# constantinpape/torch-em

Measured on AMD Instinct MI355X. Metric: voxels/sec fwd+bwd, UNet3d 1x128^3 bs=2, higher is better.
Workload: dtype f32-class (forward convs on normalised activations: fp32 operands split into 2 fp16 terms = 22 mantissa bits, lo plane scaled by 2^12 with its own fp32 accumulator, 3 fp16 MFMAs per product; other forward convs 3 bf16 terms / 6 MFMAs; data-gradient convs 2 bf16 terms / 3 MFMAs (16-bit products); WEI

## Files before the change

torch_em_amd/csrc/capi.hip:

```cpp
#include "tem_common.h"
#include "conv_internal.h"
#include "tem_act.h"
#include <stdarg.h>
#include <string.h>

static thread_local char g_err[512] = "";

void tem_set_error(const char* fmt, ...) {
    va_list ap;
    va_start(ap, fmt);
    vsnprintf(g_err, sizeof(g_err), fmt, ap);
    va_end(ap);
}

extern "C" const char* tem_last_error(void) { return g_err; }

struct TemOption {
    const char* name;
    long long def;
};
static const TemOption g_opt_table[TEM_OPT_COUNT] = {
    {"wgrad_zs", 3},
    {"wgrad_zs_persist", 1},
    {"wgrad_sums", 1},
    {"wgrad_sums_min_mb", 128},
    {"fwd_persistent", -1},
    {"conv_fwd_variant", -1},
    {"conv1x1_stream", 1},
    {"fwd_ksplit_chunks", 0},
    {"wgrad_cus", 256},
    {"upsample_generic", 0},
    {"team_min_units", 0},
    {"zr_splitk", 1},
    {"zr_wide", 1},
    {"zr_tile_blocks", 1},
    {"dice_vox", 1},
    {"upsample2_ch8", 1},
    {"pool_vec8", 2},
    {"fp32_zr", 1},
    {"zr_pair", 1},
};
static long long g_opt_val[TEM_OPT_COUNT];
static bool g_opt_set[TEM_OPT_COUNT];

long long tem_option(int id) {
    if (id < 0 || id >= TEM_OPT_COUNT) return 0;
    return __atomic_load_n(&g_opt_set[id], __ATOMIC_RELAXED) ? __atomic_load_n(&g_opt_val[id], __ATOMIC_RELAXED)
                                                            : g_opt_table[id].def;
}
static int opt_find(const char* name) {
    if (!name) return -1;
    for (int i = 0; i < TEM_OPT_COUNT; ++i)
        if (!strcmp(name, g_opt_table[i].name)) return i;
    return -1;
}
extern "C" int tem_set_option(const char* name, int64_t value) {
    const int id = opt_find(name);
    TEM_REQUIRE(id >= 0, "tem_set_option: unknown option '%s'", name ? name : "(null)");
    __atomic_store_n(&g_opt_val[id], (long long)value, __ATOMIC_RELAXED);
    __atomic_store_n(&g_opt_set[id], true, __ATOMIC_RELAXED);
    return TEM_OK;
}
extern "C" int tem_get_option(const char* name, int64_t* value) {
    const int id = opt_find(name);
    TEM_REQUIRE(id >= 0 && value, "tem_get_option: unknown option '%s'", name ? name : "(null)");
    *value = (int64_t)tem_option(id);
    return TEM_OK;
}
extern "C" int tem_version(void) { return 100; }

extern "C" int tem_device_cus(void) {
    int dev = 0;
    if (hipGetDevice(&dev) != hipSuccess) return TEM_ELAUNCH;
    hipDeviceProp_t prop;
    if (hipGetDeviceProperties(&prop, dev) != hipSuccess) return TEM_ELAUNCH;
    return prop.multiProcessorCount;
}
int tem_ncu() {
    static int ncu = 0;
    if (!ncu) {
        ncu = tem_device_cus();
        if (ncu <= 0) ncu = 256;
    }
    return ncu;
}

#define TT_V 64
#define TT_C 32

__global__ __launch_bounds__(256) void k_nchw_to_nhwc(const float* __restrict__ src, float* __restrict__ dst,
                                                      int64_t dst_ld, int C, int64_t V, int64_t vtiles, int ctiles) {
    __shared__ float tile[TT_C][TT_V + 1];
    int64_t ntiles = vtiles * ctiles;
    int n = blockIdx.y;
    for (int64_t t = blockIdx.x; t < ntiles; t += gridDim.x) {
        int ct = (int)(t % ctiles);
        int64_t vt = t / ctiles;
        int64_t v0 = vt * TT_V;
        int c0 = ct * TT_C;
        for (int i = threadIdx.x; i < TT_C * TT_V; i += 256) {
            int c = i / TT_V, v = i % TT_V;
            float val = 0.f;
            if (c0 + c < C && v0 + v < V) val = src[((int64_t)n * C + c0 + c) * V + v0 + v];
            tile[c][v] = val;
        }
        __syncthreads();
        for (int i = threadIdx.x; i < TT_C * TT_V; i += 256) {
            int v = i / TT_C, c = i % TT_C;
            if (c0 + c < C && v0 + v < V) dst[((int64_t)n * V + v0 + v) * dst_ld + c0 + c] = tile[c][v];
        }
        __syncthreads();
    }
}

__global__ __launch_bounds__(256) void k_nhwc_to_nchw(const float* __restrict__ src, int64_t src_ld,
                                                      float* __restrict__ dst, int C, int64_t V, int64_t vtiles,
                                                      int ctiles) {
    __shared__ float tile[TT_C][TT_V + 1];
    int64_t ntiles = vtiles * ctiles;
    int n = blockIdx.y;
    for (int64_t t = blockIdx.x; t < ntiles; t += gridDim.x) {
        int ct = (int)(t % ctiles);
        int64_t vt = t / ctiles;
        int64_t v0 = vt * TT_V;
        int c0 = ct * TT_C;
        for (int i = threadIdx.x; i < TT_C * TT_V; i += 256) {
            int v = i / TT_C, c = i % TT_C;
            float val = 0.f;
            if (c0 + c < C && v0 + v < V) val = src[((int64_t)n * V + v0 + v) * src_ld + c0 + c];
            tile[c][v] = val;
        }
        __syncthreads();
        for (int i = threadIdx.x; i < TT_C * TT_V; i += 256) {
            int c = i / TT_V, v = i % TT_V;
            if (c0 + c < C && v0 + v < V) dst[((int64_t)n * C + c0 + c) * V + v0 + v] = tile[c][v];
        }
        __syncthreads();
    }
}

extern "C" int tem_nchw_to_nhwc(const float* src, float* dst, int64_t dst_ld, int N, int C, int64_t V,
                                tem_stream_t stream) {
    TEM_REQUIRE(src && dst && N > 0 && C > 0 && V > 0 && dst_ld >= C, "tem_nchw_to_nhwc: bad arguments");
    int64_t vtiles = tem_cdiv(V, TT_V);
    int ctiles = (int)tem_cdiv(C, TT_C);
    int64_t nt = vtiles * ctiles;
    dim3 grid((unsigned)(nt > 4096 ? 4096 : nt), N);
    hipLaunchKernelGGL(k_nchw_to_nhwc, grid, dim3(256), 0, (hipStream_t)stream, src, dst, dst_ld, C, V, vtiles, ctiles);
    TEM_CHECK_LAUNCH("tem_nchw_to_nhwc");
    return TEM_OK;
}

extern "C" int tem_nhwc_to_nchw(const float* src, int64_t src_ld, float* dst, int N, int C, int64_t V,
                                tem_stream_t stream) {
    TEM_REQUIRE(src && dst && N > 0 && C > 0 && V > 0 && src_ld >= C, "tem_nhwc_to_nchw: bad arguments");
    int64_t vtiles = tem_cdiv(V, TT_V);
    int ctiles = (int)tem_cdiv(C, TT_C);
    int64_t nt = vtiles * ctiles;
    dim3 grid((unsigned)(nt > 4096 ? 4096 : nt), N);
    hipLaunchKernelGGL(k_nhwc_to_nchw, grid, dim3(256), 0, (hipStream_t)stream, src, src_ld, dst, C, V, vtiles, ctiles);
    TEM_CHECK_LAUNCH("tem_nhwc_to_nchw");
    return TEM_OK;
}

#define STD_BLOCKS 256

__global__ __launch_bounds__(256) void k_std_partial(const float* __restrict__ x, int64_t L, double* __restrict__ part) {
    int n = blockIdx.y;
    const float* row = x + (int64_t)n * L;
    double s = 0.0, ss = 0.0;
    for (int64_t i = (int64_t)blockIdx.x * 256 + threadIdx.x; i < L; i += (int64_t)gridDim.x * 256) {
        double v = (double)row[i];
        s += v;
        ss += v * v;
    }
    s = tem_wave_sum_d(s);
    ss = tem_wave_sum_d(ss);
    __shared__ double sh[2][4];
    int w = threadIdx.x >> 6;
    if ((threadIdx.x & 63) == 0) { sh[0][w] = s; sh[1][w] = ss; }
    __syncthreads();
    if (threadIdx.x == 0) {
        part[((int64_t)n * gridDim.x + blockIdx.x) * 2 + 0] = sh[0][0] + sh[0][1] + sh[0][2] + sh[0][3];
        part[((int64_t)n * gridDim.x + blockIdx.x) * 2 + 1] = sh[1][0] + sh[1][1] + sh[1][2] + sh[1][3];
    }
}

__global__ __launch_bounds__(256) void k_std_apply(const float* __restrict__ x, float* __restrict__ y, int64_t L,
                                                   const double* __restrict__ part, int nblk, float eps) {
    int n = blockIdx.y;
    __shared__ float sh_mean, sh_inv;
    if (threadIdx.x == 0) {
        double s = 0.0, ss = 0.0;
// ... 49 lines not shown
```

torch_em_amd/csrc/pool_upsample.hip:

```cpp
#include "tem_common.h"
#include "tem_act.h"

template <int VEC>
struct VecT;
template <>
struct VecT<4> {
    typedef float4 type;
};
template <>
struct VecT<1> {
    typedef float type;
};

template <int VEC, typename T>
__device__ __forceinline__ void ld_vec(const T* p, float (&v)[VEC]) {
    if constexpr (VEC == 8) {
        act_ld8(p, v);
    } else if constexpr (VEC == 4) {
        const float4 t = act_ld4(p);
        v[0] = t.x; v[1] = t.y; v[2] = t.z; v[3] = t.w;
    } else {
        v[0] = act_ld1(p);
    }
}
// ... 744 lines not shown
    if constexpr (CH == 8) act_st8(p, a.v);
    else act_st4(p, make_float4(a.v[0], a.v[1], a.v[2], a.v[3]));
}
template <int CH>
__device__ __forceinline__ FV<CH> fv_zero() {
    FV<CH> r;
#pragma unroll
    for (int j = 0; j < CH; ++j) r.v[j] = 0.f;
    return r;
}
template <int CH>
__device__ __forceinline__ FV<CH> lerp2(float l0, const FV<CH>& a, float l1, const FV<CH>& b) {
    FV<CH> r;
#pragma unroll
    for (int j = 0; j < CH; ++j) r.v[j] = l0 * a.v[j] + l1 * b.v[j];
    return r;
}

template <int FZ, typename T, int CH = 4>
__global__ __launch_bounds__(256) void k_upsample2_fwd(const T* __restrict__ x, int64_t x_ld, T* __restrict__ y,
                                                       int64_t y_ld, int D, int H, int W, int C,
                                                       float* __restrict__ part) {
    extern __shared__ float lsu[];
    const int Ho = 2 * H, Wo = 2 * W;
    const int cq = C / CH;
    int row = blockIdx.x;
    const int yi = row % H;
    row /= H;
    const int zi = row % D;
    const int n = row / D;
    const int ym = max(yi - 1, 0), yp = min(yi + 1, H - 1);
    const int zm = max(zi - 1, 0), zp = min(zi + 1, D - 1);
    const float ya0 = yi == 0 ? 1.f : 0.25f, ya1 = yi == 0 ? 0.f : 0.75f;
    const float za0 = zi == 0 ? 1.f : 0.25f, za1 = zi == 0 ? 0.f : 0.75f;
    const int zrow[3] = {zm, zi, zp}, yrow[3] = {ym, yi, yp};
    float s1[CH], s2[CH];
#pragma unroll
    for (int j = 0; j < CH; ++j) s1[j] = s2[j] = 0.f;
    for (int i = threadIdx.x; i < W * cq; i += 256) {
        const int xi = i / cq, c0 = (i % cq) * CH;
        const int xm = max(xi - 1, 0), xp = min(xi + 1, W - 1);
        const float xa0 = xi == 0 ? 1.f : 0.25f, xa1 = xi == 0 ? 0.f : 0.75f;
        FV<CH> Y[FZ == 2 ? 3 : 1][2][2];
#pragma unroll
        for (int kz = 0; kz < (FZ == 2 ? 3 : 1); ++kz) {
            const int zc = FZ == 2 ? zrow[kz] : zi;
            FV<CH> X[3][2];
#pragma unroll
            for (int ky = 0; ky < 3; ++ky) {
                const T* r = x + ((((int64_t)n * D + zc) * H + yrow[ky]) * W) * x_ld + c0;
                const FV<CH> a = ldv<CH>(r + (int64_t)xm * x_ld), b = ldv<CH>(r + (int64_t)xi * x_ld), c = ldv<CH>(r + (int64_t)xp * x_ld);
                X[ky][0] = lerp2(xa0, a, xa1, b);
                X[ky][1] = lerp2(0.75f, b, 0.25f, c);
            }
#pragma unroll
            for (int sx = 0; sx < 2; ++sx) {
                Y[kz][0][sx] = lerp2(ya0, X[0][sx], ya1, X[1][sx]);
                Y[kz][1][sx] = lerp2(0.75f, X[1][sx], 0.25f, X[2][sx]);
            }
            __builtin_amdgcn_sched_barrier(0);
        }
#pragma unroll
        for (int sz = 0; sz < FZ; ++sz)
#pragma unroll
            for (int sy = 0; sy < 2; ++sy)
#pragma unroll
                for (int sx = 0; sx < 2; ++sx) {
                    FV<CH> o;
                    if constexpr (FZ == 2)
                        o = sz == 0 ? lerp2(za0, Y[0][sy][sx], za1, Y[1][sy][sx]) : lerp2(0.75f, Y[1][sy][sx], 0.25f, Y[2][sy][sx]);
                    else
                        o = Y[0][sy][sx];
                    const int64_t vo = (((int64_t)n * (D * FZ) + zi * FZ + sz) * Ho + 2 * yi + sy) * Wo + 2 * xi + sx;
                    if constexpr (sizeof(T) == 2) {
#pragma unroll
                        for (int j = 0; j < CH; j += 2) {
                            const unsigned pk = act_pk<T>(o.v[j], o.v[j + 1]);
                            o.v[j] = act_lo<T>(pk);
                            o.v[j + 1] = act_hi<T>(pk);
                        }
                    }
                    stv<CH>(y + vo * y_ld + c0, o);
#pragma unroll
                    for (int j = 0; j < CH; ++j) {
                        s1[j] += o.v[j];
                        s2[j] = fmaf(o.v[j], o.v[j], s2[j]);
                    }
                }
    }
    if (part) {
        const int wv = threadIdx.x >> 6, lane = threadIdx.x & 63;
#pragma unroll
        for (int j = 0; j < CH; ++j) {
            for (int o = cq; o < 64; o <<= 1) {
                s1[j] += __shfl_xor(s1[j], o, 64);
                s2[j] += __shfl_xor(s2[j], o, 64);
            }
            if (lane < cq) {
                lsu[(wv * C + lane * CH + j) * 2 + 0] = s1[j];
                lsu[(wv * C + lane * CH + j) * 2 + 1] = s2[j];
            }
        }
        __syncthreads();
        for (int t = threadIdx.x; t < 2 * C; t += 256) {
            float a = 0.f;
            for (int w4 = 0; w4 < 4; ++w4) a += lsu[w4 * 2 * C + t];
            part[((int64_t)n * D * H + (int64_t)zi * H + yi) * 2 * C + t] = a;
        }
    }
}

struct UpbAxis {
    int idx[6];
    float w[2][4];
};
__device__ __forceinline__ UpbAxis upb_axis2(int i0, int in) {
    UpbAxis a;
    const int out = 2 * in;
#pragma unroll
    for (int k = 0; k < 6; ++k) a.idx[k] = min(max(2 * i0 - 1 + k, 0), out - 1);
#pragma unroll
    for (int c = 0; c < 2; ++c)
#pragma unroll
        for (int k = 0; k < 4; ++k) {
            const int o = 2 * i0 - 1 + 2 * c + k;
            a.w[c][k] = (o >= 0 && o < out && i0 + c < in) ? lin_w(o, 2, in, i0 + c) : 0.f;
        }
    return a;
}
__device__ __forceinline__ float upb_w(int o, int in, int i) {
    return (o >= 0 && o < 2 * in && i < in) ? lin_w(o, 2, in, i) : 0.f;
}
__device__ __forceinline__ float pick3(const float (&a)[3], int d) {
    return d == 0 ? a[0] : d == 1 ? a[1] : d == 2 ? a[2] : 0.f;
}
struct UtuAxis {
    int idx[4];
    float a[2][3];
    float s[2];
};
__device__ __forceinline__ UtuAxis utu_axis2(int i0, int f, int in) {
    UtuAxis r;
#pragma unroll
    for (int k = 0; k < 4; ++k) r.idx[k] = min(max(i0 - 1 + k, 0), in - 1);
#pragma unroll
    for (int c = 0; c < 2; ++c) {
        r.a[c][0] = r.a[c][1] = r.a[c][2] = 0.f;
        r.s[c] = 0.f;
        if (i0 + c < in) utu_axis(i0 + c, f, in, r.a[c], r.s[c]);
    }
    return r;
}

template <int FZ, typename T, int CH = 4>
__global__ __launch_bounds__(256) void k_upsample2_bwd(const T* __restrict__ gy, int64_t gy_ld,
                                                       T* __restrict__ gx, int64_t gx_ld, int D, int H, int W, int C,
                                                       const T* __restrict__ u, int64_t u_ld,
                                                       const float* __restrict__ ncoef, int64_t ncoef_ld) {
    constexpr int CZ = FZ == 2 ? 2 : 1;
    constexpr int NZF = FZ == 2 ? 6 : 1;
    const int Do = D * FZ, Ho = 2 * H, Wo = 2 * W;
    const int cq = C / CH;
    const int Hp = (H + 1) >> 1, Wp = (W + 1) >> 1, Dp = (D + CZ - 1) / CZ;
    int row = blockIdx.x;
    const int y0 = (row % Hp) * 2;
    row /= Hp;
    const int z0 = (row % Dp) * CZ;
    const int n = row / Dp;
    for (int i = threadIdx.x; i < Wp * cq; i += 256) {
        const int x0 = (i / cq) * 2, c0 = (i % cq) * CH;
        const UpbAxis ax = upb_axis2(x0, W);
        FV<CH> acc[CZ][2][2];
#pragma unroll
        for (int a = 0; a < CZ; ++a)
#pragma unroll
            for (int b = 0; b < 2; ++b)
#pragma unroll
                for (int c = 0; c < 2; ++c) acc[a][b][c] = fv_zero<CH>();
#pragma unroll 1
        for (int kz = 0; kz < NZF; ++kz) {
            const int oz = FZ == 2 ? 2 * z0 - 1 + kz : z0;
            const int zf = min(max(oz, 0), Do - 1);
            float wz[CZ];
#pragma unroll
            for (int a = 0; a < CZ; ++a) wz[a] = FZ == 2 ? upb_w(oz, D, z0 + a) : 1.f;
            FV<CH> pp[2][2];
#pragma unroll
            for (int b = 0; b < 2; ++b)
#pragma unroll
                for (int c = 0; c < 2; ++c) pp[b][c] = fv_zero<CH>();
#pragma unroll 2
            for (int ky = 0; ky < 6; ++ky) {
                const int oy = 2 * y0 - 1 + ky;
                const float wy[2] = {upb_w(oy, H, y0), upb_w(oy, H, y0 + 1)};
                const T* r = gy + ((((int64_t)n * Do + zf) * Ho + min(max(oy, 0), Ho - 1)) * Wo) * gy_ld + c0;
                FV<CH> t[6];
#pragma unroll
                for (int kx = 0; kx < 6; ++kx) t[kx] = ldv<CH>(r + (int64_t)ax.idx[kx] * gy_ld);
#pragma unroll
                for (int c = 0; c < 2; ++c)
#pragma unroll
                    for (int j = 0; j < CH; ++j) {
                        const float xr = ax.w[c][0] * t[2 * c].v[j] + ax.w[c][1] * t[2 * c + 1].v[j] +
                                         ax.w[c][2] * t[2 * c + 2].v[j] + ax.w[c][3] * t[2 * c + 3].v[j];
                        pp[0][c].v[j] = fmaf(wy[0], xr, pp[0][c].v[j]);
                        pp[1][c].v[j] = fmaf(wy[1], xr, pp[1][c].v[j]);
                    }
            }
#pragma unroll
            for (int a = 0; a < CZ; ++a)
#pragma unroll
                for (int b = 0; b < 2; ++b)
#pragma unroll
                    for (int c = 0; c < 2; ++c)
#pragma unroll
                        for (int j = 0; j < CH; ++j) acc[a][b][c].v[j] = fmaf(wz[a], pp[b][c].v[j], acc[a][b][c].v[j]);
        }
        if (ncoef) {
            const UtuAxis bx = utu_axis2(x0, 2, W), by = utu_axis2(y0, 2, H), bz = utu_axis2(z0, FZ, D);
            FV<CH> q[CZ][2][2];
#pragma unroll
            for (int a = 0; a < CZ; ++a)
#pragma unroll
                for (int b = 0; b < 2; ++b)
#pragma unroll
                    for (int c = 0; c < 2; ++c) q[a][b][c] = fv_zero<CH>();
            constexpr int NZU = FZ == 2 ? 4 : 1;
#pragma unroll 1
            for (int kz = 0; kz < NZU; ++kz) {
                const int zc = FZ == 2 ? min(max(z0 - 1 + kz, 0), D - 1) : z0;
                float wz[CZ];
#pragma unroll
                for (int a = 0; a < CZ; ++a) wz[a] = FZ == 2 ? pick3(bz.a[a], kz - a) : 1.f;
                FV<CH> qp[2][2];
#pragma unroll
                for (int b = 0; b < 2; ++b)
#pragma unroll
                    for (int c = 0; c < 2; ++c) qp[b][c] = fv_zero<CH>();
#pragma unroll 2
                for (int ky = 0; ky < 4; ++ky) {
                    const float wy[2] = {pick3(by.a[0], ky), pick3(by.a[1], ky - 1)};
                    const T* r = u + ((((int64_t)n * D + zc) * H + min(max(y0 - 1 + ky, 0), H - 1)) * W) * u_ld + c0;
                    FV<CH> t[4];
#pragma unroll
                    for (int kx = 0; kx < 4; ++kx) t[kx] = ldv<CH>(r + (int64_t)bx.idx[kx] * u_ld);
#pragma unroll
                    for (int c = 0; c < 2; ++c)
#pragma unroll
                        for (int j = 0; j < CH; ++j) {
                            const float xr = bx.a[c][0] * t[c].v[j] + bx.a[c][1] * t[c + 1].v[j] + bx.a[c][2] * t[c + 2].v[j];
                            qp[0][c].v[j] = fmaf(wy[0], xr, qp[0][c].v[j]);
                            qp[1][c].v[j] = fmaf(wy[1], xr, qp[1][c].v[j]);
                        }
                }
#pragma unroll
                for (int a = 0; a < CZ; ++a)
#pragma unroll
                    for (int b = 0; b < 2; ++b)
#pragma unroll
                        for (int c = 0; c < 2; ++c)
#pragma unroll
                            for (int j = 0; j < CH; ++j) q[a][b][c].v[j] = fmaf(wz[a], qp[b][c].v[j], q[a][b][c].v[j]);
            }
            float4 kc[CH];
#pragma unroll
            for (int j = 0; j < CH; ++j) kc[j] = *reinterpret_cast<const float4*>(ncoef + (int64_t)n * ncoef_ld + (c0 + j) * 4);
#pragma unroll
            for (int a = 0; a < CZ; ++a)
#pragma unroll
                for (int b = 0; b < 2; ++b)
#pragma unroll
                    for (int c = 0; c < 2; ++c) {
                        const float S = (FZ == 2 ? bz.s[a] : 1.f) * by.s[b] * bx.s[c];
#pragma unroll
                        for (int j = 0; j < CH; ++j)
                            acc[a][b][c].v[j] = kc[j].x * acc[a][b][c].v[j] - kc[j].y * S - kc[j].z * (q[a][b][c].v[j] - kc[j].w * S);
                    }
        }
#pragma unroll
        for (int a = 0; a < CZ; ++a)
#pragma unroll
            for (int b = 0; b < 2; ++b)
#pragma unroll
                for (int c = 0; c < 2; ++c) {
                    if (z0 + a >= D || y0 + b >= H || x0 + c >= W) continue;
                    const int64_t v = (((int64_t)n * D + z0 + a) * H + y0 + b) * W + x0 + c;
                    stv<CH>(gx + v * gx_ld + c0, acc[a][b][c]);
                }
    }
}

template <int VEC, typename T>
__global__ __launch_bounds__(256) void k_upsample_stats(const T* __restrict__ u, int64_t u_ld, int D, int H, int W,
                                                        int C, int fz, int fy, int fx, float* __restrict__ part) {
    extern __shared__ float lsu[];
    const int cq = C / VEC;
    int row = blockIdx.x;
    const int yi = row % H;
    row /= H;
    const int zi = row % D;
    const int n = row / D;
    float az[3], ay[3], sz, sy;
    utu_axis(zi, fz, D, az, sz);
    utu_axis(yi, fy, H, ay, sy);
    float s1[VEC], s2[VEC];
#pragma unroll
    for (int j = 0; j < VEC; ++j) s1[j] = s2[j] = 0.f;
    for (int i = threadIdx.x; i < W * cq; i += 256) {
        const int xi = i / cq, c0 = (i % cq) * VEC;
        float ax[3], sx;
        utu_axis(xi, fx, W, ax, sx);
        const float S = sz * sy * sx;
        float q[VEC], uc[VEC];
#pragma unroll
        for (int j = 0; j < VEC; ++j) q[j] = 0.f;
        ld_vec<VEC>(u + ((((int64_t)n * D + zi) * H + yi) * W + xi) * u_ld + c0, uc);
#pragma unroll
        for (int dz = -1; dz <= 1; ++dz) {
            const int zc = min(max(zi + dz, 0), D - 1);
            float t[3][3][VEC];
#pragma unroll
            for (int dy = -1; dy <= 1; ++dy) {
                const int yc = min(max(yi + dy, 0), H - 1);
#pragma unroll
                for (int dx = -1; dx <= 1; ++dx) {
                    const int xc = min(max(xi + dx, 0), W - 1);
                    ld_vec<VEC>(u + ((((int64_t)n * D + zc) * H + yc) * W + xc) * u_ld + c0, t[dy + 1][dx + 1]);
                }
            }
#pragma unroll
            for (int dy = -1; dy <= 1; ++dy)
#pragma unroll
                for (int dx = -1; dx <= 1; ++dx) {
                    const float wq = az[dz + 1] * ay[dy + 1] * ax[dx + 1];
#pragma unroll
                    for (int j = 0; j < VEC; ++j) q[j] = fmaf(wq, t[dy + 1][dx + 1][j], q[j]);
                }
        }
#pragma unroll
        for (int j = 0; j < VEC; ++j) {
            s1[j] = fmaf(S, uc[j], s1[j]);
            s2[j] = fmaf(uc[j], q[j], s2[j]);
        }
    }
    const int wv = threadIdx.x >> 6, lane = threadIdx.x & 63;
#pragma unroll
    for (int j = 0; j < VEC; ++j) {
        for (int o = cq; o < 64; o <<= 1) {
            s1[j] += __shfl_xor(s1[j], o, 64);
            s2[j] += __shfl_xor(s2[j], o, 64);
        }
        if (lane < cq) {
            lsu[(wv * C + lane * VEC + j) * 2 + 0] = s1[j];
            lsu[(wv * C + lane * VEC + j) * 2 + 1] = s2[j];
        }
    }
    __syncthreads();
    for (int t = threadIdx.x; t < 2 * C; t += 256) {
        float a = 0.f;
        for (int w4 = 0; w4 < 4; ++w4) a += lsu[w4 * 2 * C + t];
        part[((int64_t)n * D * H + (int64_t)zi * H + yi) * 2 * C + t] = a;
    }
}

static int upsample_stats_impl(const void* u, int64_t u_ld, int N, int D, int H, int W, int C, int fz, int fy, int fx,
                               float* part, int st, tem_stream_t stream) {
    TEM_REQUIRE(u && part && N > 0 && C > 0 && u_ld >= C && D > 0 && H > 0 && W > 0 && fz > 0 && fy > 0 && fx > 0,
                "tem_upsample_stats: bad arguments");
    TEM_REQUIRE(st >= 0 && st <= 2, "tem_upsample_stats: unknown storage type %d", st);
    const int cq = C / 4;
    TEM_REQUIRE(C % 4 == 0 && cq <= 64 && (cq & (cq - 1)) == 0 && u_ld % 4 == 0 && ((uintptr_t)u % tem_st_align4(st) == 0),
                "tem_upsample_stats: needs C = 4 * 2^k <= 256 channels, rows aligned to 4 elements (got C=%d)", C);
    int64_t rows = (int64_t)N * D * H;
    TEM_REQUIRE(rows < (1ll << 31), "tem_upsample_stats: too many rows");
    TEM_ST_SWITCH(st, T, hipLaunchKernelGGL((k_upsample_stats<4, T>), dim3((unsigned)rows), dim3(256), (size_t)4 * C * 2 * sizeof(float),
                                            (hipStream_t)stream, (const T*)u, u_ld, D, H, W, C, fz, fy, fx, part));
    TEM_CHECK_LAUNCH("tem_upsample_stats");
    return TEM_OK;
}
extern "C" int tem_upsample_stats(const float* u, int64_t u_ld, int N, int D, int H, int W, int C, int fz, int fy, int fx,
                                  float* part, tem_stream_t stream) {
    return upsample_stats_impl(u, u_ld, N, D, H, W, C, fz, fy, fx, part, 0, stream);
}
extern "C" int tem_upsample_stats_st(const void* u, int64_t u_ld, int N, int D, int H, int W, int C, int fz, int fy, int fx,
                                     float* part, int st, tem_stream_t stream) {
    return upsample_stats_impl(u, u_ld, N, D, H, W, C, fz, fy, fx, part, st, stream);
}

static inline bool upsample2_ok(int C, int fz, int fy, int fx) {
    return fy == 2 && fx == 2 && (fz == 1 || fz == 2) && C % 4 == 0 && !tem_option(TEM_OPT_UPSAMPLE_GENERIC);
}

extern "C" int tem_upsample_fwd_stats_ok(int C, int fz, int fy, int fx) {
    const int cq = C / 4;
    return upsample2_ok(C, fz, fy, fx) && cq <= 64 && (cq & (cq - 1)) == 0;
}

enum { UPS_GATHER1 = 0, UPS_GATHER4 = 1, UPS_FACTOR2_CH4 = 2, UPS_FACTOR2_CH8 = 3 };

static int upsample_fwd_select(const void* x, int64_t x_ld, const void* y, int64_t y_ld, int C, int fz, int fy, int fx, int st) {
    if (fz == 1 && upsample2_ok(C, fz, fy, fx) && vec8_ok(C, {x, y}, {x_ld, y_ld}, st) && ((C / 8) & (C / 8 - 1)) == 0 && C / 8 <= 64)
        return UPS_FACTOR2_CH8;
    const bool v4 = vec4_ok(C, {x, y}, {x_ld, y_ld}, st);
    if (upsample2_ok(C, fz, fy, fx) && v4) return UPS_FACTOR2_CH4;
    return v4 ? UPS_GATHER4 : UPS_GATHER1;
}

extern "C" int tem_upsample_fwd_path(const void* x, int64_t x_ld, const void* y, int64_t y_ld, int N, int D, int H, int W, int C,
                                     int fz, int fy, int fx, int has_part, int st) {
    if (!(x && y && N > 0 && C > 0 && x_ld >= C && y_ld >= C && D > 0 && H > 0 && W > 0 && fz > 0 && fy > 0 && fx > 0)) return -1;
    if (st < 0 || st > 2 || (int64_t)N * D * fz * H * fy >= (1ll << 31)) return -1;
    if (has_part && !(tem_upsample_fwd_stats_ok(C, fz, fy, fx) && vec4_ok(C, {x, y}, {x_ld, y_ld}, st))) return -1;
    return upsample_fwd_select(x, x_ld, y, y_ld, C, fz, fy, fx, st);
}

static int upsample_fwd_impl(const void* x, int64_t x_ld, void* y, int64_t y_ld, int N, int D, int H, int W, int C, int fz,
                             int fy, int fx, float* part, int st, tem_stream_t stream) {
    TEM_REQUIRE(x && y && N > 0 && C > 0 && x_ld >= C && y_ld >= C && D > 0 && H > 0 && W > 0,
                "tem_upsample_fwd: bad arguments");
    TEM_REQUIRE(st >= 0 && st <= 2, "tem_upsample_fwd: unknown storage type %d", st);
    TEM_REQUIRE(fz > 0 && fy > 0 && fx > 0, "tem_upsample_fwd: bad factors");
    const bool v4 = vec4_ok(C, {x, y}, {x_ld, y_ld}, st);
    TEM_REQUIRE(!part || (tem_upsample_fwd_stats_ok(C, fz, fy, fx) && v4),
                "tem_upsample_fwd_stats: needs factors (1|2, 2, 2), C = 4 * 2^k <= 256 and rows aligned to 4 elements");
    int64_t rows = (int64_t)N * D * fz * H * fy;
    TEM_REQUIRE(rows < (1ll << 31), "tem_upsample_fwd: too many rows");
    const size_t ldsb = part ? (size_t)4 * C * 2 * sizeof(float) : 0;
    const int path = upsample_fwd_select(x, x_ld, y, y_ld, C, fz, fy, fx, st);
    if (path == UPS_FACTOR2_CH8) {
        const int64_t crow = (int64_t)N * D * H;
        TEM_ST16_SWITCH(st, T, {
            hipLaunchKernelGGL((k_upsample2_fwd<1, T, 8>), dim3((unsigned)crow), dim3(256), ldsb, (hipStream_t)stream, (const T*)x,
                               x_ld, (T*)y, y_ld, D, H, W, C, part);
        });
        TEM_CHECK_LAUNCH("tem_upsample_fwd");
        return TEM_OK;
    }
    TEM_ST_SWITCH(st, T, {
        const T* xs = (const T*)x;
        T* ys = (T*)y;
        if (path == UPS_FACTOR2_CH4) {
            const int64_t crow = (int64_t)N * D * H;
            if (fz == 2)
                hipLaunchKernelGGL((k_upsample2_fwd<2, T>), dim3((unsigned)crow), dim3(256), ldsb, (hipStream_t)stream, xs, x_ld, ys,
                                   y_ld, D, H, W, C, part);
            else
                hipLaunchKernelGGL((k_upsample2_fwd<1, T>), dim3((unsigned)crow), dim3(256), ldsb, (hipStream_t)stream, xs, x_ld, ys,
                                   y_ld, D, H, W, C, part);
        } else if (path == UPS_GATHER4)
            hipLaunchKernelGGL((k_upsample_fwd<4, T>), dim3((unsigned)rows), dim3(256), 0, (hipStream_t)stream, xs, x_ld, ys,
                               y_ld, D, H, W, C, fz, fy, fx);
        else
            hipLaunchKernelGGL((k_upsample_fwd<1, T>), dim3((unsigned)rows), dim3(256), 0, (hipStream_t)stream, xs, x_ld, ys,
                               y_ld, D, H, W, C, fz, fy, fx);
    });
    TEM_CHECK_LAUNCH("tem_upsample_fwd");
    return TEM_OK;
}

extern "C" int tem_upsample_fwd_stats(const float* x, int64_t x_ld, float* y, int64_t y_ld, int N, int D, int H, int W,
                                      int C, int fz, int fy, int fx, float* part, tem_stream_t stream) {
    TEM_REQUIRE(part, "tem_upsample_fwd_stats: bad arguments");
    return upsample_fwd_impl(x, x_ld, y, y_ld, N, D, H, W, C, fz, fy, fx, part, 0, stream);
}

extern "C" int tem_upsample_fwd(const float* x, int64_t x_ld, float* y, int64_t y_ld, int N, int D, int H, int W, int C,
                                int fz, int fy, int fx, tem_stream_t stream) {
    return upsample_fwd_impl(x, x_ld, y, y_ld, N, D, H, W, C, fz, fy, fx, nullptr, 0, stream);
}

extern "C" int tem_upsample_fwd_st(const void* x, int64_t x_ld, void* y, int64_t y_ld, int N, int D, int H, int W, int C,
                                   int fz, int fy, int fx, float* part, int st, tem_stream_t stream) {
    return upsample_fwd_impl(x, x_ld, y, y_ld, N, D, H, W, C, fz, fy, fx, part, st, stream);
}

static int upsample_bwd_select(const void* gy, int64_t gy_ld, const void* gx, int64_t gx_ld, int N, int D, int H, int W, int C,
                               int fz, int fy, int fx, const void* u, int64_t u_ld, int st) {
    const int64_t pairs = (int64_t)N * ((D + fz - 1) / fz) * ((H + 1) / 2) * ((W + 1) / 2) * (C / 4);
    if (upsample2_ok(C, fz, fy, fx) && pairs >= 2 * 65536 && vec8_ok(C, {gy, gx, u}, {gy_ld, gx_ld, u ? u_ld : 0}, st) && tem_option(TEM_OPT_UPSAMPLE2_CH8))
        return UPS_FACTOR2_CH8;
    if (upsample2_ok(C, fz, fy, fx) && pairs >= 65536 && vec4_ok(C, {gy, gx, u}, {gy_ld, gx_ld, u_ld}, st)) return UPS_FACTOR2_CH4;
    return vec4_ok(C, {gy, gx, u}, {gy_ld, gx_ld, u ? u_ld : 0}, st) ? UPS_GATHER4 : UPS_GATHER1;
}

extern "C" int tem_upsample_bwd_path(const void* gy, int64_t gy_ld, const void* gx, int64_t gx_ld, int N, int D, int H, int W, int C,
                                     int fz, int fy, int fx, const void* u, int64_t u_ld, int st) {
    if (!(gy && gx && N > 0 && C > 0 && gy_ld >= C && gx_ld >= C && D > 0 && H > 0 && W > 0 && fz > 0 && fy > 0 && fx > 0)) return -1;
    if (st < 0 || st > 2 || (int64_t)N * D * H >= (1ll << 31)) return -1;
    if (u && !(u_ld >= C && (C % 4 || (u_ld % 4 == 0 && (uintptr_t)u % tem_st_align4(st) == 0)))) return -1;
    return upsample_bwd_select(gy, gy_ld, gx, gx_ld, N, D, H, W, C, fz, fy, fx, u, u_ld, st);
}

static int upsample_bwd_impl(const void* gy, int64_t gy_ld, void* gx, int64_t gx_ld, int N, int D, int H, int W,
                             int C, int fz, int fy, int fx, const void* u, int64_t u_ld, const float* ncoef,
                             int64_t ncoef_ld, int st, tem_stream_t stream) {
    TEM_REQUIRE(gy && gx && N > 0 && C > 0 && gy_ld >= C && gx_ld >= C && D > 0 && H > 0 && W > 0,
                "tem_upsample_bwd: bad arguments");
    TEM_REQUIRE(st >= 0 && st <= 2, "tem_upsample_bwd: unknown storage type %d", st);
    TEM_REQUIRE(fz > 0 && fy > 0 && fx > 0, "tem_upsample_bwd: bad factors");
    int64_t rows = (int64_t)N * D * H;
    TEM_REQUIRE(rows < (1ll << 31), "tem_upsample_bwd: too many rows");
    const int path = upsample_bwd_select(gy, gy_ld, gx, gx_ld, N, D, H, W, C, fz, fy, fx, u, u_ld, st);
    if (path == UPS_FACTOR2_CH8) {
        TEM_ST16_SWITCH(st, T, {
            if (fz == 2) {
                const int64_t prow = (int64_t)N * ((D + 1) / 2) * ((H + 1) / 2);
                hipLaunchKernelGGL((k_upsample2_bwd<2, T, 8>), dim3((unsigned)prow), dim3(256), 0, (hipStream_t)stream, (const T*)gy,
                                   gy_ld, (T*)gx, gx_ld, D, H, W, C, (const T*)u, u_ld, ncoef, ncoef_ld);
            } else {
                const int64_t prow = (int64_t)N * D * ((H + 1) / 2);
                hipLaunchKernelGGL((k_upsample2_bwd<1, T, 8>), dim3((unsigned)prow), dim3(256), 0, (hipStream_t)stream, (const T*)gy,
                                   gy_ld, (T*)gx, gx_ld, D, H, W, C, (const T*)u, u_ld, ncoef, ncoef_ld);
            }
        });
        TEM_CHECK_LAUNCH("tem_upsample_bwd");
        return TEM_OK;
    }
    TEM_ST_SWITCH(st, T, {
        const T* gys = (const T*)gy;
        const T* us = (const T*)u;
        T* gxs = (T*)gx;
        if (path == UPS_FACTOR2_CH4) {
            if (fz == 2) {
                const int64_t prow = (int64_t)N * ((D + 1) / 2) * ((H + 1) / 2);
                hipLaunchKernelGGL((k_upsample2_bwd<2, T>), dim3((unsigned)prow), dim3(256), 0, (hipStream_t)stream, gys, gy_ld, gxs,
                                   gx_ld, D, H, W, C, us, u_ld, ncoef, ncoef_ld);
            } else {
                const int64_t prow = (int64_t)N * D * ((H + 1) / 2);
                hipLaunchKernelGGL((k_upsample2_bwd<1, T>), dim3((unsigned)prow), dim3(256), 0, (hipStream_t)stream, gys, gy_ld, gxs,
                                   gx_ld, D, H, W, C, us, u_ld, ncoef, ncoef_ld);
            }
        } else if (path == UPS_GATHER4)
            hipLaunchKernelGGL((k_upsample_bwd<4, T>), dim3((unsigned)rows), dim3(256), 0, (hipStream_t)stream, gys, gy_ld, gxs,
                               gx_ld, D, H, W, C, fz, fy, fx, us, u_ld, ncoef, ncoef_ld);
        else
            hipLaunchKernelGGL((k_upsample_bwd<1, T>), dim3((unsigned)rows), dim3(256), 0, (hipStream_t)stream, gys, gy_ld, gxs,
                               gx_ld, D, H, W, C, fz, fy, fx, us, u_ld, ncoef, ncoef_ld);
    });
    TEM_CHECK_LAUNCH("tem_upsample_bwd");
    return TEM_OK;
}

extern "C" int tem_upsample_bwd(const float* gy, int64_t gy_ld, float* gx, int64_t gx_ld, int N, int D, int H, int W,
                                int C, int fz, int fy, int fx, tem_stream_t stream) {
    return upsample_bwd_impl(gy, gy_ld, gx, gx_ld, N, D, H, W, C, fz, fy, fx, nullptr, 0, nullptr, 0, 0, stream);
}

extern "C" int tem_upsample_bwd_norm(const float* gy, int64_t gy_ld, float* gx, int64_t gx_ld, int N, int D, int H,
                                     int W, int C, int fz, int fy, int fx, const float* u, int64_t u_ld,
                                     const float* ncoef, int64_t ncoef_ld, tem_stream_t stream) {
    TEM_REQUIRE(u && ncoef, "tem_upsample_bwd_norm: bad arguments");
    return tem_upsample_bwd_st(gy, gy_ld, gx, gx_ld, N, D, H, W, C, fz, fy, fx, u, u_ld, ncoef, ncoef_ld, TEM_ST_F32, stream);
}

extern "C" int tem_upsample_bwd_st(const void* gy, int64_t gy_ld, void* gx, int64_t gx_ld, int N, int D, int H, int W, int C,
                                   int fz, int fy, int fx, const void* u, int64_t u_ld, const float* ncoef, int64_t ncoef_ld,
                                   int st, tem_stream_t stream) {
    TEM_REQUIRE((u == nullptr) == (ncoef == nullptr), "tem_upsample_bwd_norm: u and ncoef come together");
    if (ncoef) {
        TEM_REQUIRE(u_ld >= C && ncoef_ld >= 4 * C && ((uintptr_t)ncoef % 16 == 0) && ncoef_ld % 4 == 0,
                    "tem_upsample_bwd_norm: bad arguments");
        TEM_REQUIRE(st >= 0 && st <= 2 && (C % 4 || (u_ld % 4 == 0 && (uintptr_t)u % tem_st_align4(st) == 0)),
                    "tem_upsample_bwd_norm: u must be aligned to 4 elements");
    }
    return upsample_bwd_impl(gy, gy_ld, gx, gx_ld, N, D, H, W, C, fz, fy, fx, u, u_ld, ncoef, ncoef_ld, st, stream);
}
```

torch_em_amd/csrc/tem_common.h:

```cpp
#pragma once
#include <hip/hip_runtime.h>
#include <stdint.h>
#include <stdio.h>
#include "../../include/tem_hip.h"

void tem_set_error(const char* fmt, ...);

enum {
    TEM_OPT_WGRAD_ZS = 0,
    TEM_OPT_WGRAD_ZS_PERSIST,
    TEM_OPT_WGRAD_SUMS,
    TEM_OPT_WGRAD_SUMS_MIN_MB,
    TEM_OPT_FWD_PERSISTENT,
    TEM_OPT_CONV_FWD_VARIANT,
    TEM_OPT_CONV1X1_STREAM,
    TEM_OPT_FWD_KSPLIT_CHUNKS,
    TEM_OPT_WGRAD_CUS,
    TEM_OPT_UPSAMPLE_GENERIC,
    TEM_OPT_TEAM_MIN_UNITS,
    TEM_OPT_ZR_SPLITK,
    TEM_OPT_ZR_WIDE,
    TEM_OPT_ZR_TILE_BLOCKS,
    TEM_OPT_DICE_VOX,
    TEM_OPT_UPSAMPLE2_CH8,
    TEM_OPT_POOL_VEC8,
    TEM_OPT_FP32_ZR,
    TEM_OPT_ZR_PAIR,
    TEM_OPT_COUNT
};
long long tem_option(int id);
int tem_ncu();

#define TEM_REQUIRE(cond, ...)                 \
    do {                                       \
        if (!(cond)) {                         \
            tem_set_error(__VA_ARGS__);        \
            return TEM_EINVAL;                 \
        }                                      \
    } while (0)

#define TEM_TRY(call)                          \
    do {                                       \
        const int rc__ = (call);               \
        if (rc__ != TEM_OK) return rc__;       \
    } while (0)

#define TEM_CHECK_LAUNCH(name)                                                   \
    do {                                                                         \
        hipError_t e__ = hipGetLastError();                                      \
        if (e__ != hipSuccess) {                                                 \
            tem_set_error("%s: launch failed: %s", name, hipGetErrorString(e__)); \
            return TEM_ELAUNCH;                                                  \
        }                                                                        \
    } while (0)

static inline int64_t tem_cdiv(int64_t a, int64_t b) { return (a + b - 1) / b; }
static inline int64_t tem_align_up(int64_t a, int64_t b) { return tem_cdiv(a, b) * b; }

static inline int tem_grid_1d(int64_t work_items, int block, int max_blocks = 256 * 8) {
    int64_t g = tem_cdiv(work_items, block);
    if (g > max_blocks) g = max_blocks;
    if (g < 1) g = 1;
    return (int)g;
}

#define TEM_WAVE 64

__device__ __forceinline__ float tem_amax4(float m, float a, float b, float c, float d) {
    return __builtin_fmaxf(__builtin_fmaxf(m, __builtin_fmaxf(__builtin_fabsf(a), __builtin_fabsf(b))),
                           __builtin_fmaxf(__builtin_fabsf(c), __builtin_fabsf(d)));
}
__device__ __forceinline__ void tem_amax_commit(unsigned* amax, float m) {
    unsigned u = __builtin_bit_cast(unsigned, m);
#pragma unroll
    for (int o = 32; o > 0; o >>= 1) u = max(u, (unsigned)__shfl_xor((int)u, o, 64));
    if ((threadIdx.x & 63) == 0 && u > __atomic_load_n(amax, __ATOMIC_RELAXED)) atomicMax(amax, u);
}

__device__ __forceinline__ float tem_wave_sum(float v) {
#pragma unroll
    for (int o = 32; o > 0; o >>= 1) v += __shfl_xor(v, o, 64);
    return v;
}
__device__ __forceinline__ double tem_wave_sum_d(double v) {
#pragma unroll
    for (int o = 32; o > 0; o >>= 1) v += __shfl_xor(v, o, 64);
    return v;
}

__device__ __forceinline__ int tem_xcd_remap(int bid, int nwg) {
    const int nx = 8;
    int q = nwg / nx, r = nwg % nx;
    int xcd = bid % nx, idx = bid / nx;
    int base = (xcd < r) ? xcd * (q + 1) : r * (q + 1) + (xcd - r) * q;
    return base + idx;
}
```

Measured before the change: 279.6 million.

## Add z-marching upsample2 backward kernel that reuses shared gradient planes across pairs

Adds a new trilinear-upsample backward kernel in which each thread walks along z through a segment of depth pairs. The two output-gradient planes shared by consecutive pairs are loaded once and folded into both accumulators, instead of being re-read by a separate block. Blocks are also retiled as 2D x/y tiles, and the grid is split into z segments sized to reach at least 512 blocks. The aim is to cut redundant global loads of the upsampled gradient, at the cost of more registers (a second accumulator set) and less parallelism along z.

After: 279.7 million, median of 3. About the same (+0.0%).

```diff
diff --git a/torch_em_amd/csrc/capi.hip b/torch_em_amd/csrc/capi.hip
--- a/torch_em_amd/csrc/capi.hip
+++ b/torch_em_amd/csrc/capi.hip
@@ -39,6 +39,7 @@
     {"pool_vec8", 2},
     {"fp32_zr", 1},
     {"zr_pair", 1},
+    {"upsample2_bwd_march", 1},
 };
 static long long g_opt_val[TEM_OPT_COUNT];
 static bool g_opt_set[TEM_OPT_COUNT];
diff --git a/torch_em_amd/csrc/pool_upsample.hip b/torch_em_amd/csrc/pool_upsample.hip
--- a/torch_em_amd/csrc/pool_upsample.hip
+++ b/torch_em_amd/csrc/pool_upsample.hip
@@ -920,6 +920,135 @@
     return r;
 }
 
+template <int CH>
+__device__ __forceinline__ void upb_fold_row(const FV<CH> (&t)[6], const float (&w)[2][4], const float (&wy)[2], FV<CH> (&pp)[2][2]) {
+#pragma unroll
+    for (int c = 0; c < 2; ++c)
+#pragma unroll
+        for (int j = 0; j < CH; ++j) {
+            const float xr = w[c][0] * t[2 * c].v[j] + w[c][1] * t[2 * c + 1].v[j] + w[c][2] * t[2 * c + 2].v[j] +
+                             w[c][3] * t[2 * c + 3].v[j];
+            pp[0][c].v[j] = fmaf(wy[0], xr, pp[0][c].v[j]);
+            pp[1][c].v[j] = fmaf(wy[1], xr, pp[1][c].v[j]);
+        }
+}
+template <int CZ, int CH>
+__device__ __forceinline__ void upb_fold_plane(const float (&wz)[CZ], const FV<CH> (&pp)[2][2], FV<CH> (&acc)[CZ][2][2]) {
+#pragma unroll
+    for (int a = 0; a < CZ; ++a)
+#pragma unroll
+        for (int b = 0; b < 2; ++b)
+#pragma unroll
+            for (int c = 0; c < 2; ++c)
+#pragma unroll
+                for (int j = 0; j < CH; ++j) acc[a][b][c].v[j] = fmaf(wz[a], pp[b][c].v[j], acc[a][b][c].v[j]);
+}
+
+template <typename T, int CH>
+__device__ __forceinline__ void upb_plane(const T* __restrict__ gy, int64_t gy_ld, int64_t plane, int y0, int H, int W, int c0,
+                                          const UpbAxis& ax, FV<CH> (&pp)[2][2]) {
+    const int Ho = 2 * H, Wo = 2 * W;
+#pragma unroll
+    for (int b = 0; b < 2; ++b)
+#pragma unroll
+        for (int c = 0; c < 2; ++c) pp[b][c] = fv_zero<CH>();
+#pragma unroll 2
+    for (int ky = 0; ky < 6; ++ky) {
+        const int oy = 2 * y0 - 1 + ky;
+        const float wy[2] = {upb_w(oy, H, y0), upb_w(oy, H, y0 + 1)};
+        const T* r = gy + ((plane * Ho + min(max(oy, 0), Ho - 1)) * Wo) * gy_ld + c0;
+        FV<CH> t[6];
+#pragma unroll
+        for (int kx = 0; kx < 6; ++kx) t[kx] = ldv<CH>(r + (int64_t)ax.idx[kx] * gy_ld);
+        upb_fold_row<CH>(t, ax.w, wy, pp);
+    }
+}
+
+template <int FZ, typename T, int CH>
+__device__ __forceinline__ void upb_norm_q(FV<CH> (&q)[FZ == 2 ? 2 : 1][2][2], const T* __restrict__ u, int64_t u_ld, int n, int z0,
+                                           int y0, int x0, int c0, int D, int H, int W) {
+    constexpr int CZ = FZ == 2 ? 2 : 1;
+    const UtuAxis bx = utu_axis2(x0, 2, W), by = utu_axis2(y0, 2, H), bz = utu_axis2(z0, FZ, D);
+#pragma unroll
+    for (int a = 0; a < CZ; ++a)
+#pragma unroll
+        for (int b = 0; b < 2; ++b)
+#pragma unroll
+            for (int c = 0; c < 2; ++c) q[a][b][c] = fv_zero<CH>();
+    constexpr int NZU = FZ == 2 ? 4 : 1;
+#pragma unroll 1
+    for (int kz = 0; kz < NZU; ++kz) {
+        const int zc = FZ == 2 ? min(max(z0 - 1 + kz, 0), D - 1) : z0;
+        float wz[CZ];
+#pragma unroll
+        for (int a = 0; a < CZ; ++a) wz[a] = FZ == 2 ? pick3(bz.a[a], kz - a) : 1.f;
+        FV<CH> qp[2][2];
+#pragma unroll
+        for (int b = 0; b < 2; ++b)
+#pragma unroll
+            for (int c = 0; c < 2; ++c) qp[b][c] = fv_zero<CH>();
+#pragma unroll 2
+        for (int ky = 0; ky < 4; ++ky) {
+            const float wy[2] = {pick3(by.a[0], ky), pick3(by.a[1], ky - 1)};
+            const T* r = u + ((((int64_t)n * D + zc) * H + min(max(y0 - 1 + ky, 0), H - 1)) * W) * u_ld + c0;
+            FV<CH> t[4];
+#pragma unroll
+            for (int kx = 0; kx < 4; ++kx) t[kx] = ldv<CH>(r + (int64_t)bx.idx[kx] * u_ld);
+#pragma unroll
+            for (int c = 0; c < 2; ++c)
+#pragma unroll
+                for (int j = 0; j < CH; ++j) {
+                    const float xr = bx.a[c][0] * t[c].v[j] + bx.a[c][1] * t[c + 1].v[j] + bx.a[c][2] * t[c + 2].v[j];
+                    qp[0][c].v[j] = fmaf(wy[0], xr, qp[0][c].v[j]);
+                    qp[1][c].v[j] = fmaf(wy[1], xr, qp[1][c].v[j]);
+                }
+        }
+#pragma unroll
+        for (int a = 0; a < CZ; ++a)
+#pragma unroll
+            for (int b = 0; b < 2; ++b)
+#pragma unroll
+                for (int c = 0; c < 2; ++c)
+#pragma unroll
+                    for (int j = 0; j < CH; ++j) q[a][b][c].v[j] = fmaf(wz[a], qp[b][c].v[j], q[a][b][c].v[j]);
+    }
+}
+template <int FZ, typename T, int CH>
+__device__ __forceinline__ void upb_finish_pair(FV<CH> (&acc)[FZ == 2 ? 2 : 1][2][2], T* __restrict__ gx, int64_t gx_ld,
+                                                const T* __restrict__ u, int64_t u_ld, const float* __restrict__ ncoef,
+                                                int64_t ncoef_ld, int n, int z0, int y0, int x0, int c0, int D, int H, int W) {
+    constexpr int CZ = FZ == 2 ? 2 : 1;
+    if (ncoef) {
+        FV<CH> q[CZ][2][2];
+        upb_norm_q<FZ, T, CH>(q, u, u_ld, n, z0, y0, x0, c0, D, H, W);
+        const UtuAxis bx = utu_axis2(x0, 2, W), by = utu_axis2(y0, 2, H), bz = utu_axis2(z0, FZ, D);
+        float4 kc[CH];
+#pragma unroll
+        for (int j = 0; j < CH; ++j) kc[j] = *reinterpret_cast<const float4*>(ncoef + (int64_t)n * ncoef_ld + (c0 + j) * 4);
+#pragma unroll
+        for (int a = 0; a < CZ; ++a)
+#pragma unroll
+            for (int b = 0; b < 2; ++b)
+#pragma unroll
+                for (int c = 0; c < 2; ++c) {
+                    const float S = (FZ == 2 ? bz.s[a] : 1.f) * by.s[b] * bx.s[c];
+#pragma unroll
+                    for (int j = 0; j < CH; ++j)
+                        acc[a][b][c].v[j] = kc[j].x * acc[a][b][c].v[j] - kc[j].y * S - kc[j].z * (q[a][b][c].v[j] - kc[j].w * S);
+                }
+    }
+#pragma unroll
+    for (int a = 0; a < CZ; ++a)
+#pragma unroll
+        for (int b = 0; b < 2; ++b)
+#pragma unroll
+            for (int c = 0; c < 2; ++c) {
+                if (z0 + a >= D || y0 + b >= H || x0 + c >= W) continue;
+                const int64_t v = (((int64_t)n * D + z0 + a) * H + y0 + b) * W + x0 + c;
+                stv<CH>(gx + v * gx_ld + c0, acc[a][b][c]);
+            }
+}
+
 template <int FZ, typename T, int CH = 4>
 __global__ __launch_bounds__(256) void k_upsample2_bwd(const T* __restrict__ gy, int64_t gy_ld,
                                                        T* __restrict__ gx, int64_t gx_ld, int D, int H, int W, int C,
@@ -927,7 +1056,7 @@
                                                        const float* __restrict__ ncoef, int64_t ncoef_ld) {
     constexpr int CZ = FZ == 2 ? 2 : 1;
     constexpr int NZF = FZ == 2 ? 6 : 1;
-    const int Do = D * FZ, Ho = 2 * H, Wo = 2 * W;
+    const int Do = D * FZ;
     const int cq = C / CH;
     const int Hp = (H + 1) >> 1, Wp = (W + 1) >> 1, Dp = (D + CZ - 1) / CZ;
     int row = blockIdx.x;
@@ -953,108 +1082,86 @@
 #pragma unroll
             for (int a = 0; a < CZ; ++a) wz[a] = FZ == 2 ? upb_w(oz, D, z0 + a) : 1.f;
             FV<CH> pp[2][2];
+            upb_plane<T, CH>(gy, gy_ld, (int64_t)n * Do + zf, y0, H, W, c0, ax, pp);
+            upb_fold_plane<CZ, CH>(wz, pp, acc);
+        }
+        upb_finish_pair<FZ, T, CH>(acc, gx, gx_ld, u, u_ld, ncoef, ncoef_ld, n, z0, y0, x0, c0, D, H, W);
+    }
+}
+
+template <int FZ, typename T, int CH = 4>
+__global__ __launch_bounds__(256) void k_upsample2_bwd_march(const T* __restrict__ gy, int64_t gy_ld, T* __restrict__ gx, int64_t gx_ld,
+                                                             int D, int H, int W, int C, const T* __restrict__ u, int64_t u_ld,
+                                                             const float* __restrict__ ncoef, int64_t ncoef_ld, int ty, int npair,
+                                                             int nseg) {
+    constexpr int CZ = FZ == 2 ? 2 : 1;
+    const int Do = D * FZ;
+    const int cq = C / CH;
+    const int Hp = (H + 1) >> 1, Wp = (W + 1) >> 1, Dp = (D + CZ - 1) / CZ;
+    const int ix = 256 / ty;
+    const int nxt = (Wp * cq + ix - 1) / ix, nyt = (Hp + ty - 1) / ty;
+    int blk = blockIdx.x;
+    const int xt = blk % nxt;
+    blk /= nxt;
+    const int yt = blk % nyt;
+    blk /= nyt;
+    const int seg = blk % nseg;
+    const int n = blk / nseg;
+    const int i = xt * ix + (int)threadIdx.x % ix, yp = yt * ty + (int)threadIdx.x / ix;
+    if (i >= Wp * cq || yp >= Hp) return;
+    const int x0 = (i / cq) * 2, c0 = (i % cq) * CH, y0 = yp * 2;
+    const UpbAxis ax = upb_axis2(x0, W);
+    const int zp0 = seg * npair, zp1 = min(zp0 + npair, Dp);
+    FV<CH> acc[CZ][2][2];
+#pragma unroll
+    for (int a = 0; a < CZ; ++a)
+#pragma unroll
+        for (int b = 0; b < 2; ++b)
+#pragma unroll
+            for (int c = 0; c < 2; ++c) acc[a][b][c] = fv_zero<CH>();
+#pragma unroll 1
+    for (int zp = zp0; zp < zp1; ++zp) {
+        const int z0 = zp * CZ;
+        if constexpr (FZ == 2) {
+            const bool more = zp + 1 < zp1;
+            FV<CH> nxa[CZ][2][2];
+#pragma unroll
+            for (int a = 0; a < CZ; ++a)
+#pragma unroll
+                for (int b = 0; b < 2; ++b)
+#pragma unroll
+                    for (int c = 0; c < 2; ++c) nxa[a][b][c] = fv_zero<CH>();
+#pragma unroll 1
+            for (int kz = zp == zp0 ? 0 : 2; kz < 6; ++kz) {
+                const int oz = 2 * z0 - 1 + kz;
+                const int zf = min(max(oz, 0), Do - 1);
+                FV<CH> pp[2][2];
+                upb_plane<T, CH>(gy, gy_ld, (int64_t)n * Do + zf, y0, H, W, c0, ax, pp);
+                const float wz[CZ] = {upb_w(oz, D, z0), upb_w(oz, D, z0 + 1)};
+                upb_fold_plane<CZ, CH>(wz, pp, acc);
+                if (more && kz >= 4) {
+                    const float wn[CZ] = {upb_w(oz, D, z0 + 2), upb_w(oz, D, z0 + 3)};
+                    upb_fold_plane<CZ, CH>(wn, pp, nxa);
+                }
+            }
+            upb_finish_pair<FZ, T, CH>(acc, gx, gx_ld, u, u_ld, ncoef, ncoef_ld, n, z0, y0, x0, c0, D, H, W);
+#pragma unroll
+            for (int a = 0; a < CZ; ++a)
+#pragma unroll
+                for (int b = 0; b < 2; ++b)
+#pragma unroll
+                    for (int c = 0; c < 2; ++c) acc[a][b][c] = nxa[a][b][c];
+        } else {
+            FV<CH> pp[2][2];
+            upb_plane<T, CH>(gy, gy_ld, (int64_t)n * Do + z0, y0, H, W, c0, ax, pp);
+            const float wz[CZ] = {1.f};
+            upb_fold_plane<CZ, CH>(wz, pp, acc);
+            upb_finish_pair<FZ, T, CH>(acc, gx, gx_ld, u, u_ld, ncoef, ncoef_ld, n, z0, y0, x0, c0, D, H, W);
 #pragma unroll
             for (int b = 0; b < 2; ++b)
 #pragma unroll
-                for (int c = 0; c < 2; ++c) pp[b][c] = fv_zero<CH>();
-#pragma unroll 2
-            for (int ky = 0; ky < 6; ++ky) {
-                const int oy = 2 * y0 - 1 + ky;
-                const float wy[2] = {upb_w(oy, H, y0), upb_w(oy, H, y0 + 1)};
-                const T* r = gy + ((((int64_t)n * Do + zf) * Ho + min(max(oy, 0), Ho - 1)) * Wo) * gy_ld + c0;
-                FV<CH> t[6];
-#pragma unroll
-                for (int kx = 0; kx < 6; ++kx) t[kx] = ldv<CH>(r + (int64_t)ax.idx[kx] * gy_ld);
-#pragma unroll
-                for (int c = 0; c < 2; ++c)
-#pragma unroll
-                    for (int j = 0; j < CH; ++j) {
-                        const float xr = ax.w[c][0] * t[2 * c].v[j] + ax.w[c][1] * t[2 * c + 1].v[j] +
-                                         ax.w[c][2] * t[2 * c + 2].v[j] + ax.w[c][3] * t[2 * c + 3].v[j];
-                        pp[0][c].v[j] = fmaf(wy[0], xr, pp[0][c].v[j]);
-                        pp[1][c].v[j] = fmaf(wy[1], xr, pp[1][c].v[j]);
-                    }
-            }
-#pragma unroll
-            for (int a = 0; a < CZ; ++a)
-#pragma unroll
-                for (int b = 0; b < 2; ++b)
-#pragma unroll
-                    for (int c = 0; c < 2; ++c)
-#pragma unroll
-                        for (int j = 0; j < CH; ++j) acc[a][b][c].v[j] = fmaf(wz[a], pp[b][c].v[j], acc[a][b][c].v[j]);
-        }
-        if (ncoef) {
-            const UtuAxis bx = utu_axis2(x0, 2, W), by = utu_axis2(y0, 2, H), bz = utu_axis2(z0, FZ, D);
-            FV<CH> q[CZ][2][2];
-#pragma unroll
-            for (int a = 0; a < CZ; ++a)
-#pragma unroll
-                for (int b = 0; b < 2; ++b)
-#pragma unroll
-                    for (int c = 0; c < 2; ++c) q[a][b][c] = fv_zero<CH>();
-            constexpr int NZU = FZ == 2 ? 4 : 1;
-#pragma unroll 1
-            for (int kz = 0; kz < NZU; ++kz) {
-                const int zc = FZ == 2 ? min(max(z0 - 1 + kz, 0), D - 1) : z0;
-                float wz[CZ];
-#pragma unroll
-                for (int a = 0; a < CZ; ++a) wz[a] = FZ == 2 ? pick3(bz.a[a], kz - a) : 1.f;
-                FV<CH> qp[2][2];
-#pragma unroll
-                for (int b = 0; b < 2; ++b)
-#pragma unroll
-                    for (int c = 0; c < 2; ++c) qp[b][c] = fv_zero<CH>();
-#pragma unroll 2
-                for (int ky = 0; ky < 4; ++ky) {
-                    const float wy[2] = {pick3(by.a[0], ky), pick3(by.a[1], ky - 1)};
-                    const T* r = u + ((((int64_t)n * D + zc) * H + min(max(y0 - 1 + ky, 0), H - 1)) * W) * u_ld + c0;
-                    FV<CH> t[4];
-#pragma unroll
-                    for (int kx = 0; kx < 4; ++kx) t[kx] = ldv<CH>(r + (int64_t)bx.idx[kx] * u_ld);
-#pragma unroll
-                    for (int c = 0; c < 2; ++c)
-#pragma unroll
-                        for (int j = 0; j < CH; ++j) {
-                            const float xr = bx.a[c][0] * t[c].v[j] + bx.a[c][1] * t[c + 1].v[j] + bx.a[c][2] * t[c + 2].v[j];
-                            qp[0][c].v[j] = fmaf(wy[0], xr, qp[0][c].v[j]);
-                            qp[1][c].v[j] = fmaf(wy[1], xr, qp[1][c].v[j]);
-                        }
-                }
-#pragma unroll
-                for (int a = 0; a < CZ; ++a)
-#pragma unroll
-                    for (int b = 0; b < 2; ++b)
-#pragma unroll
-                        for (int c = 0; c < 2; ++c)
-#pragma unroll
-                            for (int j = 0; j < CH; ++j) q[a][b][c].v[j] = fmaf(wz[a], qp[b][c].v[j], q[a][b][c].v[j]);
-            }
-            float4 kc[CH];
-#pragma unroll
-            for (int j = 0; j < CH; ++j) kc[j] = *reinterpret_cast<const float4*>(ncoef + (int64_t)n * ncoef_ld + (c0 + j) * 4);
-#pragma unroll
-            for (int a = 0; a < CZ; ++a)
-#pragma unroll
-                for (int b = 0; b < 2; ++b)
-#pragma unroll
-                    for (int c = 0; c < 2; ++c) {
-                        const float S = (FZ == 2 ? bz.s[a] : 1.f) * by.s[b] * bx.s[c];
-#pragma unroll
-                        for (int j = 0; j < CH; ++j)
-                            acc[a][b][c].v[j] = kc[j].x * acc[a][b][c].v[j] - kc[j].y * S - kc[j].z * (q[a][b][c].v[j] - kc[j].w * S);
-                    }
-        }
-#pragma unroll
-        for (int a = 0; a < CZ; ++a)
-#pragma unroll
-            for (int b = 0; b < 2; ++b)
-#pragma unroll
-                for (int c = 0; c < 2; ++c) {
-                    if (z0 + a >= D || y0 + b >= H || x0 + c >= W) continue;
-                    const int64_t v = (((int64_t)n * D + z0 + a) * H + y0 + b) * W + x0 + c;
-                    stv<CH>(gx + v * gx_ld + c0, acc[a][b][c]);
-                }
+                for (int c = 0; c < 2; ++c) acc[0][b][c] = fv_zero<CH>();
+        }
     }
 }
 
@@ -1259,6 +1366,28 @@
     return upsample_bwd_select(gy, gy_ld, gx, gx_ld, N, D, H, W, C, fz, fy, fx, u, u_ld, st);
 }
 
+struct UpbMarch {
+    int ok, fills, ty, npair, nseg;
+    int64_t blocks;
+};
+static constexpr int UPB_MARCH_BLOCKS = 512;
+static UpbMarch upb_march_geom(int N, int D, int H, int W, int C, int fz, int ch) {
+    UpbMarch g;
+    const int cq = C / ch, Hp = (H + 1) / 2, Wp = (W + 1) / 2, Dp = (D + fz - 1) / fz;
+    g.ty = 8;
+    while (g.ty > 1 && (g.ty * g.ty * cq > 256 || g.ty > Hp)) g.ty >>= 1;
+    const int ix = 256 / g.ty;
+    const int64_t cols = (int64_t)N * ((Hp + g.ty - 1) / g.ty) * (((int64_t)Wp * cq + ix - 1) / ix);
+    const int64_t want = (UPB_MARCH_BLOCKS + cols - 1) / cols, most = std::max(1, Dp / 2);
+    g.nseg = (int)std::min(want, most);
+    g.npair = (Dp + g.nseg - 1) / g.nseg;
+    g.nseg = (Dp + g.npair - 1) / g.npair;
+    g.blocks = cols * g.nseg;
+    g.ok = Hp >= 2 && (int64_t)Wp * cq * 2 >= ix && g.blocks < (1ll << 31);
+    g.fills = g.blocks >= UPB_MARCH_BLOCKS;
+    return g;
+}
+
 static int upsample_bwd_impl(const void* gy, int64_t gy_ld, void* gx, int64_t gx_ld, int N, int D, int H, int W,
                              int C, int fz, int fy, int fx, const void* u, int64_t u_ld, const float* ncoef,
                              int64_t ncoef_ld, int st, tem_stream_t stream) {
@@ -1269,9 +1398,20 @@
     int64_t rows = (int64_t)N * D * H;
     TEM_REQUIRE(rows < (1ll << 31), "tem_upsample_bwd: too many rows");
     const int path = upsample_bwd_select(gy, gy_ld, gx, gx_ld, N, D, H, W, C, fz, fy, fx, u, u_ld, st);
+    const int64_t march_opt = tem_option(TEM_OPT_UPSAMPLE2_BWD_MARCH);
     if (path == UPS_FACTOR2_CH8) {
+        const UpbMarch mg = upb_march_geom(N, D, H, W, C, fz, 8);
         TEM_ST16_SWITCH(st, T, {
-            if (fz == 2) {
+            if (mg.ok && (march_opt == 2 || (march_opt == 1 && mg.fills))) {
+                if (fz == 2)
+                    hipLaunchKernelGGL((k_upsample2_bwd_march<2, T, 8>), dim3((unsigned)mg.blocks), dim3(256), 0, (hipStream_t)stream,
+                                       (const T*)gy, gy_ld, (T*)gx, gx_ld, D, H, W, C, (const T*)u, u_ld, ncoef, ncoef_ld, mg.ty, mg.npair,
+                                       mg.nseg);
+                else
+                    hipLaunchKernelGGL((k_upsample2_bwd_march<1, T, 8>), dim3((unsigned)mg.blocks), dim3(256), 0, (hipStream_t)stream,
+                                       (const T*)gy, gy_ld, (T*)gx, gx_ld, D, H, W, C, (const T*)u, u_ld, ncoef, ncoef_ld, mg.ty, mg.npair,
+                                       mg.nseg);
+            } else if (fz == 2) {
                 const int64_t prow = (int64_t)N * ((D + 1) / 2) * ((H + 1) / 2);
                 hipLaunchKernelGGL((k_upsample2_bwd<2, T, 8>), dim3((unsigned)prow), dim3(256), 0, (hipStream_t)stream, (const T*)gy,
                                    gy_ld, (T*)gx, gx_ld, D, H, W, C, (const T*)u, u_ld, ncoef, ncoef_ld);
@@ -1289,7 +1429,15 @@
         const T* us = (const T*)u;
         T* gxs = (T*)gx;
         if (path == UPS_FACTOR2_CH4) {
-            if (fz == 2) {
+            const UpbMarch mg = upb_march_geom(N, D, H, W, C, fz, 4);
+            if (mg.ok && (march_opt == 2 || (march_opt == 1 && mg.fills))) {
+                if (fz == 2)
+                    hipLaunchKernelGGL((k_upsample2_bwd_march<2, T>), dim3((unsigned)mg.blocks), dim3(256), 0, (hipStream_t)stream, gys,
+                                       gy_ld, gxs, gx_ld, D, H, W, C, us, u_ld, ncoef, ncoef_ld, mg.ty, mg.npair, mg.nseg);
+                else
+                    hipLaunchKernelGGL((k_upsample2_bwd_march<1, T>), dim3((unsigned)mg.blocks), dim3(256), 0, (hipStream_t)stream, gys,
+                                       gy_ld, gxs, gx_ld, D, H, W, C, us, u_ld, ncoef, ncoef_ld, mg.ty, mg.npair, mg.nseg);
+            } else if (fz == 2) {
                 const int64_t prow = (int64_t)N * ((D + 1) / 2) * ((H + 1) / 2);
                 hipLaunchKernelGGL((k_upsample2_bwd<2, T>), dim3((unsigned)prow), dim3(256), 0, (hipStream_t)stream, gys, gy_ld, gxs,
                                    gx_ld, D, H, W, C, us, u_ld, ncoef, ncoef_ld);
diff --git a/torch_em_amd/csrc/tem_common.h b/torch_em_amd/csrc/tem_common.h
--- a/torch_em_amd/csrc/tem_common.h
+++ b/torch_em_amd/csrc/tem_common.h
@@ -26,6 +26,7 @@
     TEM_OPT_POOL_VEC8,
     TEM_OPT_FP32_ZR,
     TEM_OPT_ZR_PAIR,
+    TEM_OPT_UPSAMPLE2_BWD_MARCH,
     TEM_OPT_COUNT
 };
 long long tem_option(int id);
```
